# ELEKTRONN/ELEKTRONN2

Hardware: AMD Instinct MI355X
Metric: training_input_voxels_per_sec (higher is better)
Workload: dtype f32; 1 GPU; neuro3d_lite (1,1,23,183,183)->(1,2,10,37,37) fwd+bwd+Adam, 1 sample/GPU; parallelism=dp1, hipgraph=True, steps_per_launch=10

## Files before the change

elektronn2_amd/autotune.py:

```python
from __future__ import annotations

import json
import math
import os

from . import tiling
from .backend import E2Error

_HERE = os.path.dirname(os.path.abspath(__file__))
_SHIPPED = os.path.join(_HERE, "tuned.json")
_cache = None
_dirty = False
IGEMM_MTS = [1, 2, 3, 4, 5, 6, 7, 8, 10, 13]
WGRAD_MTS = [1, 2, 3, 4, 5, 7]


def _cache_path():
    return os.environ.get("E2HIP_TUNE_CACHE", os.path.join(_HERE, ".tune_cache.json"))


def _load():
    global _cache
    if _cache is None:
        _cache = {}
# ... 153 lines not shown
                    if g > 1 and (tiles <= n_cu or wm * wn > 6):
                        continue
                    cands.append("4,%d,%d,%d,%d,%d,%d,%d" % (mg, nt, cc, sk, wm, wn, g))
    return cands


def wgrad_candidates(cout, cin, k, out_sp, n_cu=256):
    mblocks = -(-cout // 16)
    T = k[0] * k[1] * k[2]
    nblocks = -(-(cin * T) // 16)
    q = out_sp[1] * out_sp[2]
    qpad = out_sp[1] * (out_sp[2] + 2 * (k[2] - 1))
    cands = []
    for mt in _best_mts(mblocks, WGRAD_MTS, keep=3):
        nmt = -(-mblocks // mt)
        variants = [(1, 1), (2, 1), (4, 1), (2, 14), (4, 14), (1, 0), (2, 0), (4, 0)]
        if nblocks <= 2:
            variants = [(1, 4), (1, 0), (1, 1), (2, 14)]
        for nt, wk in variants:
            wn = 1 if wk in (4, 14) else 4
            if nt > 1 and 16 * nt * wn > 16 * nblocks:
                continue
            nnt = -(-nblocks // (nt * wn))
            for bp in ((128, 256) if wk in (1, 14) else (64, 128)):
                tiles = out_sp[0] * (-(-(qpad if wk in (1, 14) else q) // bp))
                for fill in (1, 1.5, 2, 3, 4):
                    ps = max(1, min(tiles, int(n_cu * fill) // max(1, nmt * nnt)))
                    for q in {ps} | set(_near_divisors(tiles, ps)):
                        cands.append("%d,%d,%d,%d,%d" % (mt, nt, wk, bp, q))
                        if wk in (1, 14) and nnt >= 2 and nmt * q * nnt > 8:
                            cands.append("%d,%d,%d,%d,%d" % (mt, nt, wk + 100, bp, q))
    return sorted(set(cands) | set(pointwise_wgrad_candidates(cout, cin, k, out_sp, n_cu))
                  | set(position_split_wgrad_candidates(cout, cin, k, out_sp, n_cu))
                  | set(even_split_wgrad_candidates(cout, cin, k, out_sp, n_cu)))


WGRAD_KS_TILES = [(13, 2), (10, 2), (8, 2), (8, 4), (7, 2), (7, 4), (6, 4), (5, 4), (4, 4), (3, 4), (2, 4)]


def position_split_wgrad_candidates(cout, cin, k, out_sp, n_cu=256):
    T = k[0] * k[1] * k[2]
    if T == 1 or cout < 24:
        return []
    pitch = out_sp[2] + k[2] - 1
    if (k[1] - 1) * pitch + k[2] - 1 < 31:
        return []
    units = out_sp[0] * (-(-((out_sp[1] - 1) * pitch + out_sp[2]) // 32))
    scored = []
    for mt, nt in WGRAD_KS_TILES:
        nm, nn = -(-cout // (16 * mt)), -(-(cin * T) // (16 * nt))
        eff = (cout * cin * T) / float(nm * 16 * mt * nn * 16 * nt)
        scored.append((-eff, -mt * nt, mt, nt, nm * nn))
    scored.sort()
    out = []
    for _, _, mt, nt, tiles in scored[:4]:
        for fill in (0.5, 1, 2):
            s = max(1, min(-(-units // 4), int(n_cu * fill) // tiles))
            out.append("%d,%d,9,0,%d" % (mt, nt, s))
    return sorted(set(out))


def even_split_wgrad_candidates(cout, cin, k, out_sp, n_cu=256):
    T = k[0] * k[1] * k[2]
    if T == 1:
        if cout < 32 or cin < 32 or out_sp[0] * out_sp[1] * out_sp[2] < 32:
            return []
        tiles, form = PW_WGRAD_KS_TILES, 8
# ... 193 lines not shown
```

elektronn2_amd/csrc/conv_host.hpp:

```cpp
#pragma once
#include <stdint.h>
#include <string.h>
#include "../../include/e2hip.h"

constexpr int kE2TilingChars = 64;
struct E2Tiling {
  int n = 0;
  int v[8] = {};
};

static inline bool e2_parse_tiling(const char* s, E2Tiling* out) {
  E2Tiling t;
  *out = t;
  if (!s[0]) return true;
  if (strlen(s) >= (size_t)kE2TilingChars) return false;
  for (;;) {
    if (t.n == 8) return false;
    const bool neg = *s == '-';
    if (neg) ++s;
    if (*s < '0' || *s > '9') return false;
    int64_t x = 0;
    for (; *s >= '0' && *s <= '9'; ++s) {
      x = x * 10 + (*s - '0');
      if (x > INT32_MAX) return false;
// ... 78 lines not shown
  int kd = 0, kh = 0, kw = 0;
  int Do = 0, Ho = 0, Wo = 0;
  int64_t xsN = 0, xsC = 0, xsZ = 0, xsY = 0;
  int64_t dsN = 0, dsC = 0, dsZ = 0, dsY = 0;
  int flip = 0;
  int upR = 1;
  int accumulate = 0;
  int dy_padded = 0;
};

static inline WgradArgs wgrad_args(const e2_tensor5& x, const e2_tensor5& dy, float* dw, int kd,
                                   int kh, int kw, int accumulate, int dy_padded) {
  WgradArgs a;
  a.x = x.ptr; a.dy = dy.ptr; a.dw = dw;
  a.N = x.n; a.Cin = x.c; a.Cout = dy.c;
  a.kd = kd; a.kh = kh; a.kw = kw;
  a.Do = dy.d; a.Ho = dy.h; a.Wo = dy.w;
  a.xsN = x.sn; a.xsC = x.sc; a.xsZ = x.sd; a.xsY = x.sh;
  a.dsN = dy.sn; a.dsC = dy.sc; a.dsZ = dy.sd; a.dsY = dy.sh;
  a.flip = 1;
  a.accumulate = accumulate; a.dy_padded = dy_padded;
  return a;
}

enum E2WgradFamily { E2_WG_LDS, E2_WG_DIRECT, E2_WG_PW, E2_WG_PW_KS, E2_WG_KS };
struct E2WgradRoute {
  int family = E2_WG_LDS;
  int MT = 0, NT = 0;
  int BP = 0;
  bool wave_split = false;
  bool xcd = false;
  int splits = 0;
  int bands = 0, groups = 0;
  const char* refuse = nullptr;
};
static inline E2WgradRoute e2_wgrad_route(const int v[5], bool dy_padded) {
  E2WgradRoute r;
  const int WK = v[2], BP = v[3];
  r.MT = v[0]; r.NT = v[1]; r.splits = v[4];
  if (WK == 7) { r.family = E2_WG_PW; return r; }
  if (WK == 8 || WK == 9) {
    r.family = WK == 8 ? E2_WG_PW_KS : E2_WG_KS;
    if (BP >= 1) { r.bands = BP; r.groups = v[4]; }
    return r;
  }
  r.BP = BP;
  if (dy_padded && (WK == 1 || WK == 14 || WK == 101 || WK == 114) && (BP == 128 || BP == 256)) {
    r.family = E2_WG_DIRECT; r.wave_split = WK % 100 == 14; r.xcd = WK >= 100;
    return r;
  }
  if (WK == 14 || WK >= 100) r.refuse = "wgrad: WK=14/101/114 need the padded-gradient entry point and BP 128/256";
  else if (BP != 64 && BP != 128) r.refuse = "wgrad: BP must be 64 or 128";
  else if (!(WK == 0 || WK == 1 || (WK == 4 && r.NT == 1))) r.refuse = "wgrad: WK=4 needs NT=1";
  else r.wave_split = WK == 4;
  return r;
}
static inline const char* e2_wgrad_family_name(const E2WgradRoute& r, bool bf16) {
  switch (r.family) {
    case E2_WG_PW: return "pw_wgrad";
    case E2_WG_PW_KS: return "pw_wgrad_ks";
    case E2_WG_KS: return "wgrad_ks";
    case E2_WG_DIRECT: return bf16 ? "wgrad_direct_bf16r" : "wgrad_direct";
  }
  return "wgrad_lds";
}

static inline const char* e2_pw_wgrad_limit(const WgradArgs& a, bool bf16, int ) {
  if (!(a.kd == 1 && a.kh == 1 && a.kw == 1)) return "pointwise wgrad: the kernel is not 1x1x1";
  if (!(a.xsY == a.Wo && a.xsZ == (int64_t)a.Ho * a.Wo && a.dsY == a.Wo && a.dsZ == (int64_t)a.Ho * a.Wo))
    return "pointwise wgrad: x and dy need dense channel planes (row stride = W, plane stride = H * W)";
  if (bf16) return "pointwise wgrad: an f32 kernel, not offered in bf16 mode";
  return nullptr;
}
static inline const char* e2_wgrad_ks_limit(const WgradArgs& a, bool bf16, int input_slack) {
  const int64_t Din = a.Do + a.kd - 1, Hin = a.Ho + a.kh - 1;
// ... 25 lines not shown
```

elektronn2_amd/csrc/conv_pw_wgrad.hip:

```cpp
#include "common.hpp"
#include "wgrad_even.hpp"
#include <algorithm>
#include <type_traits>
#include <vector>
#include <cstdio>

typedef float f32x4 __attribute__((ext_vector_type(4)));

#ifdef E2_DEBUG_ENV
#define KS_STAMP(i) do { if (p.stamps && threadIdx.x == 0) p.stamps[8L * blockIdx.x + (i)] = __builtin_amdgcn_s_memtime(); } while (0)
#else
#define KS_STAMP(i) do {} while (0)
#endif

namespace {

struct PgP {
  const float* a; const float* b; float* c;
  long asN, asC, bsN, bsC;
  int N, M, Ncol, K;
  int R;
  int nMT, nNT, S;
  int stepsPerSample, steps, per;
  int rem;
  int T, kh, kw, flip, planes;
  long asZ, bsZ, bsY;
  unsigned long long* stamps;
};

__device__ __forceinline__ f32x4 pg_load(const float* row, int k, int K) {
  if (k + 3 < K) {
    f32x4 v;
    __builtin_memcpy(&v, row + k, 16);
    return v;
  }
  f32x4 v = {0.f, 0.f, 0.f, 0.f};
#pragma unroll
  for (int j = 0; j < 4; ++j)
    if (k + j < K) v[j] = row[k + j];
  return v;
}

template <int MT, int NT>
__global__ __launch_bounds__(256) void pw_wgrad_kernel(PgP p) {
  const int tid = threadIdx.x, lane = tid & 63, l15 = lane & 15, q = lane >> 4;
  const int wave = __builtin_amdgcn_readfirstlane(tid >> 6);
  const int wm = wave >> 1, wn = wave & 1;
  int b = blockIdx.x;
  const int nt = b % p.nNT; b /= p.nNT;
  const int mt = b % p.nMT;
  const int sp = b / p.nMT;
  const int m0 = (mt * 2 + wm) * 16 * MT;
  const int n0 = (nt * 2 + wn) * 16 * NT;
  const int s0 = sp * p.per, s1 = min(s0 + p.per, p.steps);

  long aoff[MT], boff[NT];
#pragma unroll
  for (int mb = 0; mb < MT; ++mb) aoff[mb] = (long)min(m0 + 16 * mb + l15, p.M - 1) * p.asC;
#pragma unroll
  for (int nb = 0; nb < NT; ++nb) boff[nb] = (long)min(n0 + 16 * nb + l15, p.Ncol - 1) * p.bsC;

  f32x4 acc[MT][NT];
#pragma unroll
  for (int mb = 0; mb < MT; ++mb)
#pragma unroll
    for (int nb = 0; nb < NT; ++nb) acc[mb][nb] = f32x4{0.f, 0.f, 0.f, 0.f};

  auto load = [&](int s, f32x4 (&A)[MT], f32x4 (&B)[NT]) {
    const int sc = min(s, s1 - 1);
    const int n = sc / p.stepsPerSample;
    const int k = (sc - n * p.stepsPerSample) * 16 + 4 * q;
    const float* ap = p.a + (long)n * p.asN;
    const float* bp = p.b + (long)n * p.bsN;
#pragma unroll
    for (int mb = 0; mb < MT; ++mb) A[mb] = pg_load(ap + aoff[mb], k, p.K);
// ... 22 lines not shown
        load(s + d + D - 1, A[(d + D - 1) % D], B[(d + D - 1) % D]);
        fma(A[d], B[d]);
      }
    }
#pragma unroll
    for (int d = 0; d < D - 1; ++d)
      if (s + d < s1) fma(A[d], B[d]);
  }

  const bool single = p.S == 1;
#pragma unroll
  for (int mb = 0; mb < MT; ++mb) {
#pragma unroll
    for (int r = 0; r < 4; ++r) {
      const int m = m0 + 16 * mb + 4 * q + r;
      if (m >= p.M) continue;
      long rbase;
      int cstride;
      if (p.R > 1) { const int co = m / p.R; rbase = (long)co * p.Ncol * p.R + (m - co * p.R); cstride = p.R; }
      else { rbase = (long)m * p.Ncol; cstride = 1; }
#pragma unroll
      for (int nb = 0; nb < NT; ++nb) {
        const int n = n0 + 16 * nb + l15;
        if (n >= p.Ncol) continue;
        float* dst = p.c + rbase + (long)n * cstride;
        if (single) *dst += acc[mb][nb][r];
        else unsafeAtomicAdd(dst, acc[mb][nb][r]);
      }
    }
  }
}

template <int MT, int NT, bool TAPS>
__global__ __launch_bounds__(256) void pw_wgrad_ks_kernel(PgP p) {
  extern __shared__ float red[];
  constexpr int RW = 16 * NT + 4;
  constexpr int RS = 16 * MT * RW;
  const int tid = threadIdx.x, lane = tid & 63, l15 = lane & 15, q = lane >> 4;
  const int wave = __builtin_amdgcn_readfirstlane(tid >> 6);
  int L = blockIdx.x;
  if ((gridDim.x & 7) == 0) L = (L & 7) * (gridDim.x >> 3) + (L >> 3);
  const int nt = L % p.nNT; L /= p.nNT;
  const int mt = L % p.nMT;
  const int sp = L / p.nMT;
  const int m0 = mt * 16 * MT, n0 = nt * 16 * NT;
  const bool single = p.S == 1;
  auto dst_of = [&](int m, int n) -> float* {
    if (p.R > 1) { const int co = m / p.R; return p.c + (long)co * p.Ncol * p.R + (m - co * p.R) + (long)n * p.R; }
    return p.c + (long)m * p.Ncol + n;
  };

  if (sp >= p.S) return;
  const int u0 = sp * p.per + wave, u1 = min(sp * p.per + p.per, p.steps);
  const int cnt = u0 < u1 ? (u1 - u0 + 3) >> 2 : 0;
  KS_STAMP(0);

  unsigned aoff[MT], boff[NT];
#pragma unroll
  for (int mb = 0; mb < MT; ++mb) aoff[mb] = (unsigned)min(m0 + 16 * mb + l15, p.M - 1) * (unsigned)p.asC * 4u + 16u * q;
#pragma unroll
  for (int nb = 0; nb < NT; ++nb) {
    const int j = min(n0 + 16 * nb + l15, p.Ncol - 1);
    if (TAPS) {
      const int ci = j / p.T, ts = j - ci * p.T;
      const int t = p.flip ? p.T - 1 - ts : ts;
      const int tz = t / (p.kh * p.kw), r2 = t - tz * (p.kh * p.kw);
// ... 5 lines not shown
    }
  }

  f32x4 acc[MT][NT];
#pragma unroll
  for (int mb = 0; mb < MT; ++mb)
#pragma unroll
    for (int nb = 0; nb < NT; ++nb) acc[mb][nb] = f32x4{0.f, 0.f, 0.f, 0.f};

  auto where = [&](int i, const char*& ap, const char*& bp, unsigned& kb, unsigned& zb) {
    const int u = u0 + 4 * i;
    const int pl = u / p.stepsPerSample;
    kb = (unsigned)(u - pl * p.stepsPerSample) * 128u;
    if (TAPS) {
      const int n = pl / p.planes, z = pl - n * p.planes;
      ap = reinterpret_cast<const char*>(p.a + (long)n * p.asN + (long)z * p.asZ);
      bp = reinterpret_cast<const char*>(p.b + (long)n * p.bsN);
      zb = (unsigned)(z * p.bsZ) * 4u;
    } else {
      ap = reinterpret_cast<const char*>(p.a + (long)pl * p.asN);
      bp = reinterpret_cast<const char*>(p.b + (long)pl * p.bsN);
      zb = 0;
    }
  };
  auto bo = [&](int nb, unsigned kb, unsigned zb) -> unsigned {
    return TAPS ? boff[nb] + zb + kb : boff[nb] + kb;
  };
  auto load2 = [&](f32x4 (&d)[2], const char* base, unsigned off) {
    const char* r = base + off;
    __builtin_memcpy(&d[0], r, 16);
    __builtin_memcpy(&d[1], r + 64, 16);
  };

  if (cnt > 0) {
    f32x4 A[MT][2], Bc[NT][2], Bn[NT][2];
    const char *ap, *bp;
    unsigned kb, zb;
    where(0, ap, bp, kb, zb);
#pragma unroll
    for (int nb = 0; nb < NT; ++nb) load2(Bc[nb], bp, bo(nb, kb, zb));
#pragma unroll
    for (int mb = 0; mb < MT; ++mb) load2(A[mb], ap, aoff[mb] + kb);
    KS_STAMP(1);
#pragma unroll 1
    for (int i = 0; i < cnt; ++i) {
      where(min(i + 1, cnt - 1), ap, bp, kb, zb);
#pragma unroll
      for (int nb = 0; nb < NT; ++nb) load2(Bn[nb], bp, bo(nb, kb, zb));
#pragma unroll
      for (int mb = 0; mb < MT; ++mb) {
#pragma unroll
        for (int h = 0; h < 2; ++h)
#pragma unroll
          for (int j = 0; j < 4; ++j)
#pragma unroll
            for (int nb = 0; nb < NT; ++nb)
              acc[mb][nb] = __builtin_amdgcn_mfma_f32_16x16x4f32(A[mb][h][j], Bc[nb][h][j], acc[mb][nb], 0, 0, 0);
        load2(A[mb], ap, aoff[mb] + kb);
        __builtin_amdgcn_sched_barrier(0);
      }
#pragma unroll
      for (int nb = 0; nb < NT; ++nb) { Bc[nb][0] = Bn[nb][0]; Bc[nb][1] = Bn[nb][1]; }
#ifdef E2_DEBUG_ENV
      if (i == 0) KS_STAMP(2);
#endif
    }
  }
// ... 26 lines not shown
#pragma unroll
            for (int nb = 0; nb < NT; ++nb)
              acc[mb][nb] = __builtin_amdgcn_mfma_f32_16x16x4f32(av[mb >> 2][e], bv[nb][e], acc[mb][nb], 0, 0, 0);
        }
    }
  }

  float* mine = red + wave * RS;
#pragma unroll
  for (int mb = 0; mb < MT; ++mb)
#pragma unroll
    for (int nb = 0; nb < NT; ++nb)
#pragma unroll
      for (int r = 0; r < 4; ++r) mine[(16 * mb + 4 * q + r) * RW + 16 * nb + l15] = acc[mb][nb][r];
  __syncthreads();
  KS_STAMP(4);
#pragma unroll 2
  for (int e = tid; e < 16 * MT * 16 * NT; e += 256) {
    const int ml = e / (16 * NT), nl = e - ml * (16 * NT);
    const int m = m0 + ml, n = n0 + nl;
    const float* s = red + ml * RW + nl;
    const float v = (s[0] + s[RS]) + (s[2 * RS] + s[3 * RS]);
    if (m >= p.M || n >= p.Ncol) continue;
    float* dst = dst_of(m, n);
    if (single) *dst += v;
    else unsafeAtomicAdd(dst, v);
  }
  KS_STAMP(5);
#ifdef E2_DEBUG_ENV
  if (p.stamps) { __builtin_amdgcn_s_waitcnt(0); KS_STAMP(6); }
#endif
}

template <int MT, int NT, bool TAPS>
__global__ __launch_bounds__(256) void pw_wgrad_ev_kernel(PgP p, WgEven ev) {
  extern __shared__ float red[];
  constexpr int RW = 16 * NT + 4;
  constexpr int RS = 16 * MT * RW;
  const int tid = threadIdx.x, lane = tid & 63, l15 = lane & 15, q = lane >> 4;
  const int wave = __builtin_amdgcn_readfirstlane(tid >> 6);
  int g = blockIdx.x;
  if ((ev.G & 7) == 0) g = (g & 7) * (ev.G >> 3) + (g >> 3);
  WgRange rg = wg_even_range(ev, g);
  if (rg.b >= rg.e) return;
  KS_STAMP(0);
#ifdef E2_DEBUG_ENV
  int nseg = 0;
#endif
#pragma unroll 1
  do {
    const WgSeg sg = wg_even_seg(ev, rg);
    const int mt = sg.tile / p.nNT, nt = sg.tile - mt * p.nNT;
    const int m0 = mt * 16 * MT, n0 = nt * 16 * NT;
    const int u0 = sg.u0 + wave, u1 = sg.u0 + sg.n;
    const int cnt = u0 < u1 ? (u1 - u0 + 3) >> 2 : 0;

    unsigned aoff[MT], boff[NT];
#pragma unroll
    for (int mb = 0; mb < MT; ++mb) aoff[mb] = (unsigned)min(m0 + 16 * mb + l15, p.M - 1) * (unsigned)p.asC * 4u + 16u * q;
#pragma unroll
    for (int nb = 0; nb < NT; ++nb) {
      const int j = min(n0 + 16 * nb + l15, p.Ncol - 1);
      if (TAPS) {
        const int ci = j / p.T, ts = j - ci * p.T;
        const int t = p.flip ? p.T - 1 - ts : ts;
        const int tz = t / (p.kh * p.kw), r2 = t - tz * (p.kh * p.kw);
        const int ty = r2 / p.kw, tx = r2 - ty * p.kw;
// ... 4 lines not shown
      }
    }

    f32x4 acc[MT][NT];
#pragma unroll
    for (int mb = 0; mb < MT; ++mb)
#pragma unroll
      for (int nb = 0; nb < NT; ++nb) acc[mb][nb] = f32x4{0.f, 0.f, 0.f, 0.f};

    auto where = [&](int i, const char*& ap, const char*& bp, unsigned& kb, unsigned& zb) {
      const int u = u0 + 4 * i;
      const int pl = u / p.stepsPerSample;
      kb = (unsigned)(u - pl * p.stepsPerSample) * 128u;
      if (TAPS) {
        const int n = pl / p.planes, z = pl - n * p.planes;
        ap = reinterpret_cast<const char*>(p.a + (long)n * p.asN + (long)z * p.asZ);
        bp = reinterpret_cast<const char*>(p.b + (long)n * p.bsN);
        zb = (unsigned)(z * p.bsZ) * 4u;
      } else {
        ap = reinterpret_cast<const char*>(p.a + (long)pl * p.asN);
        bp = reinterpret_cast<const char*>(p.b + (long)pl * p.bsN);
        zb = 0;
      }
    };
    auto bo = [&](int nb, unsigned kb, unsigned zb) -> unsigned {
      return TAPS ? boff[nb] + zb + kb : boff[nb] + kb;
    };
    auto load2 = [&](f32x4 (&d)[2], const char* base, unsigned off) {
      const char* r = base + off;
      __builtin_memcpy(&d[0], r, 16);
      __builtin_memcpy(&d[1], r + 64, 16);
    };

    if (cnt > 0) {
      f32x4 A[MT][2], Bc[NT][2], Bn[NT][2];
      const char *ap, *bp;
      unsigned kb, zb;
      where(0, ap, bp, kb, zb);
#pragma unroll
      for (int nb = 0; nb < NT; ++nb) load2(Bc[nb], bp, bo(nb, kb, zb));
#pragma unroll
      for (int mb = 0; mb < MT; ++mb) load2(A[mb], ap, aoff[mb] + kb);
#pragma unroll 1
      for (int i = 0; i < cnt; ++i) {
        where(min(i + 1, cnt - 1), ap, bp, kb, zb);
#pragma unroll
        for (int nb = 0; nb < NT; ++nb) load2(Bn[nb], bp, bo(nb, kb, zb));
#pragma unroll
        for (int mb = 0; mb < MT; ++mb) {
#pragma unroll
          for (int h = 0; h < 2; ++h)
#pragma unroll
            for (int j = 0; j < 4; ++j)
#pragma unroll
              for (int nb = 0; nb < NT; ++nb)
                acc[mb][nb] = __builtin_amdgcn_mfma_f32_16x16x4f32(A[mb][h][j], Bc[nb][h][j], acc[mb][nb], 0, 0, 0);
          load2(A[mb], ap, aoff[mb] + kb);
          __builtin_amdgcn_sched_barrier(0);
        }
#pragma unroll
        for (int nb = 0; nb < NT; ++nb) { Bc[nb][0] = Bn[nb][0]; Bc[nb][1] = Bn[nb][1]; }
      }
    }
    if (!TAPS && u1 == ev.U && p.rem > 0) {
      constexpr int MBW = (MT + 3) / 4;
      const int k = p.K - p.rem + 4 * q;
#pragma unroll 1
// ... 30 lines not shown
    for (int mb = 0; mb < MT; ++mb)
#pragma unroll
      for (int nb = 0; nb < NT; ++nb)
#pragma unroll
        for (int r = 0; r < 4; ++r) mine[(16 * mb + 4 * q + r) * RW + 16 * nb + l15] = acc[mb][nb][r];
    __syncthreads();
#pragma unroll 2
    for (int e = tid; e < 16 * MT * 16 * NT; e += 256) {
      const int ml = e / (16 * NT), nl = e - ml * (16 * NT);
      const int m = m0 + ml, n = n0 + nl;
      const float* s = red + ml * RW + nl;
      const float v = (s[0] + s[RS]) + (s[2 * RS] + s[3 * RS]);
      if (m >= p.M || n >= p.Ncol) continue;
      float* dst;
      if (p.R > 1) { const int co = m / p.R; dst = p.c + (long)co * p.Ncol * p.R + (m - co * p.R) + (long)n * p.R; }
      else dst = p.c + (long)m * p.Ncol + n;
      unsafeAtomicAdd(dst, v);
    }
    __syncthreads();
#ifdef E2_DEBUG_ENV
    ++nseg;
#endif
    rg.b += sg.n;
  } while (rg.b < rg.e);
#ifdef E2_DEBUG_ENV
  if (p.stamps) {
    __builtin_amdgcn_s_waitcnt(0);
    KS_STAMP(6);
    if (threadIdx.x == 0) p.stamps[8L * blockIdx.x + 7] = (unsigned long long)nseg;
  }
#endif
}

template <int MT, int NT, bool TAPS>
int launch_ev(e2_ctx* ctx, const PgP& p, const WgEven& ev) {
  const int lds = 4 * 16 * MT * (16 * NT + 4) * (int)sizeof(float);
  static bool raised = false;
  if (int rc = e2i_raise_lds(reinterpret_cast<const void*>(&pw_wgrad_ev_kernel<MT, NT, TAPS>), lds, &raised)) return rc;
  PgP ps = p;
#ifdef E2_DEBUG_ENV
  const long grid = ev.G;
  const bool stamps = e2_dbg_env("E2_PWKS_STAMPS") != nullptr && !ctx->capturing;
  if (stamps) {
    E2_CHECK_HIP(hipMalloc(&ps.stamps, sizeof(unsigned long long) * 8 * grid));
    E2_CHECK_HIP(hipMemsetAsync(ps.stamps, 0, sizeof(unsigned long long) * 8 * grid, ctx->stream));
  }
#endif
  hipLaunchKernelGGL((pw_wgrad_ev_kernel<MT, NT, TAPS>), dim3((unsigned)ev.G), dim3(256), lds, ctx->stream, ps, ev);
  E2_CHECK_HIP(hipGetLastError());
#ifdef E2_DEBUG_ENV
  if (stamps) {
    E2_CHECK_HIP(hipStreamSynchronize(ctx->stream));
    std::vector<unsigned long long> h(8 * grid);
    E2_CHECK_HIP(hipMemcpy(h.data(), ps.stamps, sizeof(unsigned long long) * 8 * grid, hipMemcpyDeviceToHost));
    unsigned long long t0 = ~0ull, t1 = 0;
    double sum[2] = {0, 0}, mx[2] = {0, 0};
    long cntw[2] = {0, 0};
    for (long b = 0; b < grid; ++b) {
      if (!h[8 * b + 6]) continue;
      const int k = h[8 * b + 7] > 1;
      const double d = (double)(h[8 * b + 6] - h[8 * b]);
      sum[k] += d; mx[k] = std::max(mx[k], d); ++cntw[k];
      t0 = std::min(t0, h[8 * b]); t1 = std::max(t1, h[8 * b + 6]);
    }
    fprintf(stderr, "[e2] pw_wgrad_ev<%d,%d> G %d, %d tiles x %d units in %d bands, %d(+1 for %d) pairs each: first start -> last end %llu ticks\n",
            MT, NT, ev.G, ev.T, ev.U, ev.B, ev.base, ev.extra, t1 - t0);
    for (int k = 0; k < 2; ++k)
      fprintf(stderr, "   %-22s %5ld work-groups, mean %9.0f max %9.0f ticks\n", k ? "two or more segments" : "one segment",
              cntw[k], sum[k] / std::max(1L, cntw[k]), mx[k]);
    (void)hipFree(ps.stamps);
  }
#endif
  return 0;
}

static int even_split(const PgP& p, long G, int B, WgEven* ev) {
  const long T = (long)p.nMT * p.nNT;
  E2_REQUIRE(p.steps >= 1, "wgrad (even position ranges): no whole 32-position unit");
  E2_REQUIRE(T * p.steps < (1L << 31), "wgrad (even position ranges): too many (tile, unit) pairs");
  E2_REQUIRE(G >= 1 && G <= (1L << 16), "wgrad (even position ranges): %ld work-groups (1 .. 65536)", G);
  E2_REQUIRE(B >= 1 && B <= p.steps, "wgrad (even position ranges): %d bands for %d units", B, p.steps);
  *ev = wg_even_make((int)T, p.steps, (int)G, B);
  return 0;
}

template <int MT, int NT, bool TAPS>
int launch_ks(e2_ctx* ctx, const PgP& p, long grid) {
  const int lds = 4 * 16 * MT * (16 * NT + 4) * (int)sizeof(float);
  static bool raised = false;
  if (int rc = e2i_raise_lds(reinterpret_cast<const void*>(&pw_wgrad_ks_kernel<MT, NT, TAPS>), lds, &raised)) return rc;
#ifdef E2_DEBUG_ENV
  PgP ps = p;
  const bool stamps = e2_dbg_env("E2_PWKS_STAMPS") != nullptr && !ctx->capturing;
  if (stamps) {
    E2_CHECK_HIP(hipMalloc(&ps.stamps, sizeof(unsigned long long) * 8 * grid));
    E2_CHECK_HIP(hipMemsetAsync(ps.stamps, 0, sizeof(unsigned long long) * 8 * grid, ctx->stream));
  }
  hipLaunchKernelGGL((pw_wgrad_ks_kernel<MT, NT, TAPS>), dim3((unsigned)grid), dim3(256), lds, ctx->stream, ps);
  E2_CHECK_HIP(hipGetLastError());
  if (stamps) {
    E2_CHECK_HIP(hipStreamSynchronize(ctx->stream));
    std::vector<unsigned long long> h(8 * grid);
    E2_CHECK_HIP(hipMemcpy(h.data(), ps.stamps, sizeof(unsigned long long) * 8 * grid, hipMemcpyDeviceToHost));
    static const char* names[6] = {"prologue issue", "first unit", "other units", "LDS + barrier", "flush issue", "flush done"};
    double sum[6] = {0};
    unsigned long long t0 = ~0ull, t1 = 0, s1 = 0;
    long nb = 0;
    for (long b = 0; b < grid; ++b) {
      if (!h[8 * b + 6]) continue;
      ++nb;
      for (int i = 0; i < 6; ++i) sum[i] += (double)(h[8 * b + i + 1] - h[8 * b + i]);
      t0 = std::min(t0, h[8 * b]); t1 = std::max(t1, h[8 * b + 6]); s1 = std::max(s1, h[8 * b]);
    }
    fprintf(stderr, "[e2] pw_wgrad_ks<%d,%d> grid %ld (%ld main), S %d, per %d: first start -> last end %llu ticks, last start %llu\n",
            MT, NT, grid, nb, p.S, p.per, t1 - t0, s1 - t0);
    for (int i = 0; i < 6; ++i) fprintf(stderr, "   %-14s %9.0f ticks\n", names[i], sum[i] / std::max(1L, nb));
    (void)hipFree(ps.stamps);
  }
#else
  hipLaunchKernelGGL((pw_wgrad_ks_kernel<MT, NT, TAPS>), dim3((unsigned)grid), dim3(256), lds, ctx->stream, p);
  E2_CHECK_HIP(hipGetLastError());
#endif
  return 0;
}

template <int MT, int NT>
int launch(e2_ctx* ctx, const PgP& p, long grid) {
  hipLaunchKernelGGL((pw_wgrad_kernel<MT, NT>), dim3((unsigned)grid), dim3(256), 0, ctx->stream, p);
  E2_CHECK_HIP(hipGetLastError());
  return 0;
}

PgP pg_base(const WgradArgs& a, int Ncol, long K) {
  PgP p;
  p.a = a.dy; p.b = a.x; p.c = a.dw;
  p.asN = a.dsN; p.asC = a.dsC; p.bsN = a.xsN; p.bsC = a.xsC;
  p.N = a.N; p.M = a.Cout; p.Ncol = Ncol;
  p.K = (int)K;
  p.R = 1; p.rem = 0; p.stamps = nullptr;
  p.T = 1; p.kh = p.kw = 1; p.flip = 0; p.planes = 1; p.asZ = p.bsZ = p.bsY = 0;
  return p;
}

struct KsSplit { long grid; bool even; WgEven ev; };
int ks_split(e2_ctx* ctx, const WgradArgs& a, const E2WgradRoute& r, long units, const char* who, PgP& p, KsSplit* k) {
  E2_REQUIRE(units < (1L << 29), "%s: too many positions", who);
  p.steps = (int)units;
  const int S = (int)std::max<long>(1, std::min<long>(r.splits, std::max<long>(1, (units + 3) / 4)));
  p.per = (int)std::max<long>(1, (units + S - 1) / S);
  p.per = (p.per + 3) & ~3;
  p.S = (int)std::max<long>(1, (units + p.per - 1) / p.per);
  k->grid = (long)p.nMT * p.nNT * p.S;
  k->grid = (k->grid + 7) & ~7L;
  E2_REQUIRE(k->grid < (1L << 31), "%s: grid too large", who);
  k->even = r.bands >= 1;
  k->ev = WgEven{};
  if (k->even)
    if (int rc = even_split(p, r.groups, r.bands, &k->ev)) return rc;
  if (!a.accumulate)
    if (int rc = e2i_fill_flat(ctx, a.dw, (size_t)a.Cout * p.Ncol, 0.f)) return rc;
  return 0;
}
template <int MT, int NT, bool TAPS>
int launch_split(e2_ctx* ctx, const PgP& p, const KsSplit& k) {
  return k.even ? launch_ev<MT, NT, TAPS>(ctx, p, k.ev) : launch_ks<MT, NT, TAPS>(ctx, p, k.grid);
}

}

int e2i_pw_wgrad(e2_ctx* ctx, const WgradArgs& a, const E2WgradRoute& r) {
  const char* limit = e2_pw_wgrad_limit(a, ctx->mfma_bf16 != 0, ctx->input_slack);
  E2_REQUIRE(!limit, "%s", limit);
  const long K = (long)a.Do * a.Ho * a.Wo;
  E2_REQUIRE(K < (1L << 30), "pointwise wgrad: sample too large");
  PgP p = pg_base(a, a.Cin, K);
  p.R = a.upR > 1 ? a.upR : 1;
  E2_REQUIRE(a.Cout % p.R == 0, "pointwise wgrad: %d rows for %d sub-positions", a.Cout, p.R);
  p.nMT = e2_cdiv(a.Cout, 32 * r.MT);
  p.nNT = e2_cdiv(a.Cin, 32 * r.NT);
  p.stepsPerSample = (int)((K + 15) / 16);
  const long steps = (long)a.N * p.stepsPerSample;
  E2_REQUIRE(steps < (1L << 30), "pointwise wgrad: too many positions");
  p.steps = (int)steps;
  const int S = (int)std::max<long>(1, std::min<long>(r.splits, steps));
  p.per = (int)((steps + S - 1) / S);
  p.S = (int)((steps + p.per - 1) / p.per);
  const long grid = (long)p.nMT * p.nNT * p.S;
  E2_REQUIRE(grid < (1L << 31), "pointwise wgrad: grid too large");
  if (!a.accumulate)
    if (int rc = e2i_fill_flat(ctx, a.dw, (size_t)a.Cout * a.Cin, 0.f)) return rc;
#define E2_L(M, N_) if (r.MT == M && r.NT == N_) return launch<M, N_>(ctx, p, grid);
  E2_L(2, 2) E2_L(4, 2) E2_L(2, 4) E2_L(4, 4) E2_L(4, 3) E2_L(3, 4) E2_L(7, 2) E2_L(2, 7) E2_L(7, 4) E2_L(4, 7)
#undef E2_L
  e2_set_error("pointwise wgrad: no instance MT=%d NT=%d", r.MT, r.NT);
  return 2;
}

int e2i_pw_wgrad_ks(e2_ctx* ctx, const WgradArgs& a, const E2WgradRoute& r) {
  const char* limit = e2_pw_wgrad_limit(a, ctx->mfma_bf16 != 0, ctx->input_slack);
  E2_REQUIRE(!limit, "%s", limit);
  const long K = (long)a.Do * a.Ho * a.Wo;
  E2_REQUIRE(K >= 4 && K < (1L << 30), "pointwise wgrad: sample of %ld positions", K);
  E2_REQUIRE(((long)a.Cout * a.dsC + K) * 4 < (1L << 32) && ((long)a.Cin * a.xsC + K) * 4 < (1L << 32) && a.dsC >= 0 && a.xsC >= 0,
             "pointwise wgrad: sample too large for 32-bit byte offsets");
  PgP p = pg_base(a, a.Cin, K);
  p.R = a.upR > 1 ? a.upR : 1;
  E2_REQUIRE(a.Cout % p.R == 0, "pointwise wgrad: %d rows for %d sub-positions", a.Cout, p.R);
  p.nMT = e2_cdiv(a.Cout, 16 * r.MT);
  p.nNT = e2_cdiv(a.Cin, 16 * r.NT);
  p.stepsPerSample = (int)(K / 32);
  p.rem = (int)(K % 32);
  KsSplit k;
  if (int rc = ks_split(ctx, a, r, (long)a.N * p.stepsPerSample, "pointwise wgrad", p, &k)) return rc;
#define E2_L(M, N_) if (r.MT == M && r.NT == N_) return launch_split<M, N_, false>(ctx, p, k);
  E2_L(13, 2) E2_L(7, 2) E2_L(7, 4) E2_L(4, 4) E2_L(10, 2)
#undef E2_L
  e2_set_error("pointwise wgrad (position-split waves): no instance MT=%d NT=%d", r.MT, r.NT);
  return 2;
}

int e2i_wgrad_ks(e2_ctx* ctx, const WgradArgs& a, const E2WgradRoute& r) {
  const char* limit = e2_wgrad_ks_limit(a, ctx->mfma_bf16 != 0, ctx->input_slack);
  E2_REQUIRE(!limit, "%s", limit);
  const int T = a.kd * a.kh * a.kw;
  const long K = (long)(a.Ho - 1) * a.dsY + a.Wo;
  E2_REQUIRE(K >= 4 && K < (1L << 28), "wgrad (position-split GEMM): plane of %ld positions", K);
  PgP p = pg_base(a, a.Cin * T, K);
  p.T = T; p.kh = a.kh; p.kw = a.kw; p.flip = a.flip; p.planes = a.Do;
  p.asZ = a.dsZ; p.bsZ = a.xsZ; p.bsY = a.xsY;
#ifdef E2_DEBUG_ENV
  if (!ctx->capturing) {
    const int Din = a.Do + a.kd - 1, Hin = a.Ho + a.kh - 1;
    const float* end = a.x + (int64_t)(a.N - 1) * a.xsN + (int64_t)(a.Cin - 1) * a.xsC +
                       (int64_t)(Din - 1) * a.xsZ + (int64_t)(Hin - 1) * a.xsY + (a.Wo + a.kw - 1);
    float h[32];
    E2_CHECK_HIP(hipStreamSynchronize(ctx->stream));
    E2_CHECK_HIP(hipMemcpy(h, end, sizeof(h), hipMemcpyDeviceToHost));
    for (int i = 0; i < 32; ++i)
      E2_REQUIRE(h[i] == h[i] && h[i] - h[i] == 0.f, "wgrad (position-split GEMM): e2_set_input_slack promised finite "
                 "values behind x, but float %d behind its last element is %g", i, (double)h[i]);
  }
#endif
  p.nMT = e2_cdiv(a.Cout, 16 * r.MT);
  p.nNT = e2_cdiv(p.Ncol, 16 * r.NT);
  p.stepsPerSample = (int)((K + 31) / 32);
  KsSplit k;
  if (int rc = ks_split(ctx, a, r, (long)a.N * a.Do * p.stepsPerSample, "wgrad (position-split GEMM)", p, &k)) return rc;
#define E2_L(M, N_) if (r.MT == M && r.NT == N_) return launch_split<M, N_, true>(ctx, p, k);
  E2_L(13, 2) E2_L(7, 2) E2_L(7, 4) E2_L(4, 4) E2_L(10, 2) E2_L(5, 4) E2_L(3, 4) E2_L(2, 4) E2_L(8, 2) E2_L(8, 4) E2_L(6, 4)
#undef E2_L
  e2_set_error("wgrad (position-split GEMM): no instance MT=%d NT=%d", r.MT, r.NT);
  return 2;
}
```

elektronn2_amd/csrc/conv_wgrad.hip:

```cpp
#include "wgrad_common.hpp"
#include <stdlib.h>
#include <utility>

struct WgradP {
  const float* x;
  const float* dy;
  const float* zeros;
  float* dw;
  int Cin, Cout, kd, kh, kw, T, THW;
  int Do, Ho, Wo, Q;
  long xsN, xsC, xsZ, xsY;
  long dsN, dsC, dsZ, dsY;
  int flip, upR;
  int NTOT;
  int Lpad;
  int nMT, nNT, nPS;
  int nPT, tilesTotal;
  int maxSpans;
  int bufFloats;
  int Din, N;
  int dbg;
  int bf16;
  FastDiv divWo;
};
// ... 251 lines not shown
  e2_set_error("wgrad: no instance NT=%d BP=%d WK=%d", NT, BP, WK);
  return 2;
}

static int w_lpad(int Lmax) {
  return ((Lmax + 63) / 64) * 64 + 2;
}
static int w_lmax(const WgradArgs& a, int BP) {
  const int rows = (BP + a.Wo - 2) / a.Wo;
  return (BP - 1) + rows * ((int)a.xsY - a.Wo) + (a.kh - 1) * (int)a.xsY + a.kw;
}
static size_t w_buf_floats(const WgradArgs& a, int MT, int BNn, int BP) {
  const size_t dyf = (((size_t)16 * MT * (BP + 4) + 3) / 4) * 4;
  return dyf + (BP + 128) + (size_t)wg_maxspans(a, BNn) * w_lpad(w_lmax(a, BP)) + 64;
}

struct WCfg { int MT, NT, WK, BP, PS; };

static WCfg choose_wcfg(const e2_ctx* ctx, const WgradArgs& a, int* ok, int* src) {
  const int mblocks = e2_cdiv(a.Cout, 16);
  const int T = a.kd * a.kh * a.kw;
  const long NTOT = (long)a.Cin * T;
  const int nblocks = (int)((NTOT + 15) / 16);
  const long Q = (long)a.Ho * a.Wo;
  WCfg best{0, 0, 0, 0, 0};
  double bestCost = 1e300;
  const double dw_bytes = 4.0 * a.Cout * (double)NTOT;
  const E2Tiling& t = ctx->tiling_v[E2_TILING_WGRAD];
  *src = E2_SRC_MODEL;
  if (t.n) {
    *src = E2_SRC_FALLBACK;
    if (e2_wgrad_candidate(t)) {
      const WCfg f{t.v[0], t.v[1], t.v[2], t.v[3], t.v[4]};
      const char* limit = f.WK == 9 ? e2_wgrad_ks_limit(a, ctx->mfma_bf16, ctx->input_slack)
                          : (f.WK == 7 || f.WK == 8) ? e2_pw_wgrad_limit(a, ctx->mfma_bf16, ctx->input_slack)
                          : nullptr;
      if (limit == nullptr) { *ok = 1; *src = E2_SRC_FORCED; return f; }
    }
  }
  if (a.dy_padded && nblocks > 2) {
    const long S = (long)(a.Ho - 1) * a.dsY + a.Wo;
    for (int MT : kWgMTs) {
      if (MT > mblocks && MT != 1) continue;
      const int nMT = e2_cdiv(mblocks, MT);
      for (int NT = 1; NT <= 4; NT *= 2) {
        if (16 * NT * 4 > 16 * nblocks && NT > 1) continue;
        if (NT == 4 && MT * 4 >= 20) continue;
        const int nNT = e2_cdiv(nblocks, NT * 4);
        for (int BP = ctx->mfma_bf16 ? 256 : 128; BP <= 256; BP *= 2) {
          if (BP == 256 && S <= 128 && !ctx->mfma_bf16) continue;
          const size_t lds = 2 * e2i_wgrad_direct_buf_floats(a, NT, BP, 1) * 4;
          if (lds > 160 * 1024) continue;
          const int slots = ctx->num_cu;
          const int nPT = (int)((S + BP - 1) / BP);
          const long tiles = (long)a.N * a.Do * nPT;
          const long base = (long)nMT * nNT;
          for (int fill = 1; fill <= 2; ++fill) {
            long PS = std::max<long>(1, ((long)slots * fill + base - 1) / base);
            PS = std::min(PS, tiles);
            const int per = (int)((tiles + PS - 1) / PS);
            const double tile = (BP / 4.0) * MT * NT * 35.0 + (BP / 16.0) * 150.0 + 1200.0;
            const double flush = 16.0 * MT * 16.0 * NT * 4 * 0.6;
            const double wg_time = per * tile + flush + 5000.0;
            const long wgs = base * PS;
            const double rounds = (double)((wgs + slots - 1) / slots);
            const double atom = (double)PS * dw_bytes / 1.3e12 * 2.4e9 + dw_bytes / 4e12 * 2.4e9;
            const double cost = rounds * wg_time + atom;
            if (cost < bestCost) { bestCost = cost; best = WCfg{MT, NT, 1, BP, (int)PS}; }
// ... 96 lines not shown
```

elektronn2_amd/tiling.py:

```python
import re
from collections import namedtuple

_LIST = re.compile(r"-?[0-9]+(,-?[0-9]+){0,7}")


WgradRoute = namedtuple('WgradRoute', 'family MT NT WK BP wave_split xcd splits bands groups refuse')


class Tiling(namedtuple('Tiling', 'kind family v')):
    __slots__ = ()

    @property
    def WK(self):
        return wgrad_route(self, True).WK if self.family == 'wgrad' else None

    @property
    def xcd_grouped(self):
        return self.family == 'wgrad' and wgrad_route(self, True).xcd


def wgrad_route(t, dy_padded, bf16=False):
    assert t.kind == 'wgrad' and t.family == 'wgrad', t
    MT, NT, WK, BP, PS = t.v
    r = dict(family='wgrad_lds', MT=MT, NT=NT, WK=WK, BP=0, wave_split=False, xcd=False, splits=PS,
             bands=0, groups=0, refuse=None)
    if WK == 7:
        r.update(family='pw_wgrad')
    elif WK in (8, 9):
        r.update(family='pw_wgrad_ks' if WK == 8 else 'wgrad_ks')
        if BP >= 1:
            r.update(bands=BP, groups=PS)
    elif dy_padded and WK in (1, 14, 101, 114) and BP in (128, 256):
        r.update(family='wgrad_direct_bf16r' if bf16 else 'wgrad_direct', BP=BP,
                 wave_split=WK % 100 == 14, xcd=WK >= 100)
    else:
        r.update(BP=BP)
        if WK == 14 or WK >= 100:
            r.update(refuse="WK=14/101/114 need the padded-gradient entry point and BP 128/256")
        elif BP not in (64, 128):
            r.update(refuse="BP must be 64 or 128")
        elif not (WK in (0, 1) or (WK == 4 and NT == 1)):
            r.update(refuse="WK=4 needs NT=1")
        else:
            r.update(wave_split=WK == 4)
    return WgradRoute(**r)


def parse(kind, s):
    if not s or len(s) > 63 or not _LIST.fullmatch(s):
        return None
    v = tuple(int(t) for t in s.split(","))
    if any(abs(q) >= 2 ** 31 for q in v):
        return None
    fam = None
    if kind == 'igemm':
        if len(v) == 4:
            fam = '16x16x4'
        elif len(v) == 8 and v[0] == 4:
            fam = '4x4x1'
        elif len(v) in (3, 5) and v[0] == 1:
            fam = 'pointwise'
        elif len(v) >= 3 and v[0] == 32:
# ... 46 lines not shown
```

Measured before the change: 528.4 million voxels/s.

## Add six-product bf16-split wgrad variant for position-split and pointwise kernels

Adds a new wgrad kernel variant (WK=18/19) that splits each fp32 operand into three bf16 pieces and accumulates six bf16 MFMA cross-products. This gives near-fp32 accuracy on the bf16 matrix cores without the bf16 input limit checks. The new candidates are added to the autotuner's search space and routed through the existing ks/even launch paths. The cost is six MFMAs per k-step plus the splitting arithmetic, so it only helps where the autotuner finds it beats the existing fp32 paths.

```diff
diff --git a/elektronn2_amd/autotune.py b/elektronn2_amd/autotune.py
--- a/elektronn2_amd/autotune.py
+++ b/elektronn2_amd/autotune.py
@@ -209,7 +209,22 @@
                             cands.append("%d,%d,%d,%d,%d" % (mt, nt, wk + 100, bp, q))
     return sorted(set(cands) | set(pointwise_wgrad_candidates(cout, cin, k, out_sp, n_cu))
                   | set(position_split_wgrad_candidates(cout, cin, k, out_sp, n_cu))
-                  | set(even_split_wgrad_candidates(cout, cin, k, out_sp, n_cu)))
+                  | set(even_split_wgrad_candidates(cout, cin, k, out_sp, n_cu))
+                  | set(six_product_wgrad_candidates(cout, cin, k, out_sp, n_cu)))
+
+
+def six_product_form(c):
+    v = c.split(",")
+    if len(v) == 5 and v[2] in ("8", "9"):
+        return ",".join(v[:2] + ["1" + v[2]] + v[3:])
+    return None
+
+
+def six_product_wgrad_candidates(cout, cin, k, out_sp, n_cu=256):
+    out = []
+    for gen in (pointwise_wgrad_candidates, position_split_wgrad_candidates, even_split_wgrad_candidates):
+        out += [six_product_form(c) for c in gen(cout, cin, k, out_sp, n_cu)]
+    return sorted(set(c for c in out if c))
 
 
 WGRAD_KS_TILES = [(13, 2), (10, 2), (8, 2), (8, 4), (7, 2), (7, 4), (6, 4), (5, 4), (4, 4), (3, 4), (2, 4)]
diff --git a/elektronn2_amd/csrc/conv_host.hpp b/elektronn2_amd/csrc/conv_host.hpp
--- a/elektronn2_amd/csrc/conv_host.hpp
+++ b/elektronn2_amd/csrc/conv_host.hpp
@@ -134,6 +134,7 @@
   bool xcd = false;
   int splits = 0;
   int bands = 0, groups = 0;
+  bool six = false;
   const char* refuse = nullptr;
 };
 static inline E2WgradRoute e2_wgrad_route(const int v[5], bool dy_padded) {
@@ -141,8 +142,9 @@
   const int WK = v[2], BP = v[3];
   r.MT = v[0]; r.NT = v[1]; r.splits = v[4];
   if (WK == 7) { r.family = E2_WG_PW; return r; }
-  if (WK == 8 || WK == 9) {
-    r.family = WK == 8 ? E2_WG_PW_KS : E2_WG_KS;
+  if (WK == 8 || WK == 9 || WK == 18 || WK == 19) {
+    r.family = WK % 10 == 8 ? E2_WG_PW_KS : E2_WG_KS;
+    r.six = WK >= 18;
     if (BP >= 1) { r.bands = BP; r.groups = v[4]; }
     return r;
   }
diff --git a/elektronn2_amd/csrc/conv_pw_wgrad.hip b/elektronn2_amd/csrc/conv_pw_wgrad.hip
--- a/elektronn2_amd/csrc/conv_pw_wgrad.hip
+++ b/elektronn2_amd/csrc/conv_pw_wgrad.hip
@@ -41,6 +41,38 @@
   return v;
 }
 
+typedef __bf16 bf16x8 __attribute__((ext_vector_type(8)));
+typedef unsigned u32x4 __attribute__((ext_vector_type(4)));
+typedef float f32x2 __attribute__((ext_vector_type(2)));
+struct Pc3 { u32x4 p[3]; };
+
+__device__ __forceinline__ Pc3 pg_split8(const f32x4 (&d)[2]) {
+  Pc3 f;
+#pragma unroll
+  for (int h = 0; h < 2; ++h)
+#pragma unroll
+    for (int e = 0; e < 2; ++e) {
+      f32x2 r = {d[h][2 * e], d[h][2 * e + 1]};
+#pragma unroll
+      for (int pc = 0; pc < 3; ++pc) {
+        const unsigned t0 = __float_as_uint(r[0]) & 0xffff0000u, t1 = __float_as_uint(r[1]) & 0xffff0000u;
+        f.p[pc][2 * h + e] = (t0 >> 16) | t1;
+        if (pc < 2) r -= f32x2{__uint_as_float(t0), __uint_as_float(t1)};
+      }
+    }
+  return f;
+}
+template <int NT>
+__device__ __forceinline__ void pg_mfma6(const Pc3& a, const Pc3 (&b)[NT], f32x4 (&acc)[NT]) {
+  constexpr int TA[6] = {1, 0, 2, 0, 1, 0}, TB[6] = {1, 2, 0, 1, 0, 0};
+#pragma unroll
+  for (int t = 0; t < 6; ++t)
+#pragma unroll
+    for (int nb = 0; nb < NT; ++nb)
+      acc[nb] = __builtin_amdgcn_mfma_f32_16x16x32_bf16(__builtin_bit_cast(bf16x8, a.p[TA[t]]),
+                                                        __builtin_bit_cast(bf16x8, b[nb].p[TB[t]]), acc[nb], 0, 0, 0);
+}
+
 template <int MT, int NT>
 __global__ __launch_bounds__(256) void pw_wgrad_kernel(PgP p) {
   const int tid = threadIdx.x, lane = tid & 63, l15 = lane & 15, q = lane >> 4;
@@ -129,6 +161,75 @@
 }
 
 template <int MT, int NT, bool TAPS>
+__device__ __forceinline__ void pg_six_units(const PgP& p, int u0, int cnt, const unsigned (&aoff)[MT],
+                                             const unsigned (&boff)[NT], f32x4 (&acc)[MT][NT]) {
+  auto where = [&](int i, const char*& ap, const char*& bp, unsigned& kb, unsigned& zb) {
+    const int u = u0 + 4 * i;
+    const int pl = u / p.stepsPerSample;
+    kb = (unsigned)(u - pl * p.stepsPerSample) * 128u;
+    if (TAPS) {
+      const int n = pl / p.planes, z = pl - n * p.planes;
+      ap = reinterpret_cast<const char*>(p.a + (long)n * p.asN + (long)z * p.asZ);
+      bp = reinterpret_cast<const char*>(p.b + (long)n * p.bsN);
+      zb = (unsigned)(z * p.bsZ) * 4u;
+    } else {
+      ap = reinterpret_cast<const char*>(p.a + (long)pl * p.asN);
+      bp = reinterpret_cast<const char*>(p.b + (long)pl * p.bsN);
+      zb = 0;
+    }
+  };
+  auto bo = [&](int nb, unsigned kb, unsigned zb) -> unsigned {
+    return TAPS ? boff[nb] + zb + kb : boff[nb] + kb;
+  };
+  auto load2 = [&](f32x4 (&d)[2], const char* base, unsigned off) {
+    const char* r = base + off;
+    __builtin_memcpy(&d[0], r, 16);
+    __builtin_memcpy(&d[1], r + 64, 16);
+  };
+  f32x4 A[MT][2], Bn[NT][2];
+  Pc3 Ap, Bp[NT];
+  const char *ap, *bp;
+  unsigned kb, zb;
+  where(0, ap, bp, kb, zb);
+#pragma unroll
+  for (int nb = 0; nb < NT; ++nb) load2(Bn[nb], bp, bo(nb, kb, zb));
+#pragma unroll
+  for (int mb = 0; mb < MT; ++mb) load2(A[mb], ap, aoff[mb] + kb);
+#pragma unroll
+  for (int nb = 0; nb < NT; ++nb) Bp[nb] = pg_split8(Bn[nb]);
+  Ap = pg_split8(A[0]);
+  where(min(1, cnt - 1), ap, bp, kb, zb);
+#pragma unroll
+  for (int nb = 0; nb < NT; ++nb) load2(Bn[nb], bp, bo(nb, kb, zb));
+  load2(A[0], ap, aoff[0] + kb);
+#pragma unroll 1
+  for (int i = 0; i < cnt; ++i) {
+    Pc3 Bq[NT];
+#pragma unroll
+    for (int mb = 0; mb < MT; ++mb) {
+      Pc3 An;
+      if (mb + 1 < MT) {
+        An = pg_split8(A[mb + 1]);
+        load2(A[mb + 1], ap, aoff[mb + 1] + kb);
+      } else {
+        An = pg_split8(A[0]);
+#pragma unroll
+        for (int nb = 0; nb < NT; ++nb) Bq[nb] = pg_split8(Bn[nb]);
+        where(min(i + 2, cnt - 1), ap, bp, kb, zb);
+#pragma unroll
+        for (int nb = 0; nb < NT; ++nb) load2(Bn[nb], bp, bo(nb, kb, zb));
+        load2(A[0], ap, aoff[0] + kb);
+      }
+      pg_mfma6<NT>(Ap, Bp, acc[mb]);
+      Ap = An;
+      __builtin_amdgcn_sched_barrier(0);
+    }
+#pragma unroll
+    for (int nb = 0; nb < NT; ++nb) Bp[nb] = Bq[nb];
+  }
+}
+
+template <int MT, int NT, bool TAPS, bool SIX = false>
 __global__ __launch_bounds__(256) void pw_wgrad_ks_kernel(PgP p) {
   extern __shared__ float red[];
   constexpr int RW = 16 * NT + 4;
@@ -200,7 +301,9 @@
     __builtin_memcpy(&d[1], r + 64, 16);
   };
 
-  if (cnt > 0) {
+  if constexpr (SIX) {
+    if (cnt > 0) pg_six_units<MT, NT, TAPS>(p, u0, cnt, aoff, boff, acc);
+  } else if (cnt > 0) {
     f32x4 A[MT][2], Bc[NT][2], Bn[NT][2];
     const char *ap, *bp;
     unsigned kb, zb;
@@ -293,7 +396,7 @@
 #endif
 }
 
-template <int MT, int NT, bool TAPS>
+template <int MT, int NT, bool TAPS, bool SIX = false>
 __global__ __launch_bounds__(256) void pw_wgrad_ev_kernel(PgP p, WgEven ev) {
   extern __shared__ float red[];
   constexpr int RW = 16 * NT + 4;
@@ -364,7 +467,9 @@
       __builtin_memcpy(&d[1], r + 64, 16);
     };
 
-    if (cnt > 0) {
+    if constexpr (SIX) {
+      if (cnt > 0) pg_six_units<MT, NT, TAPS>(p, u0, cnt, aoff, boff, acc);
+    } else if (cnt > 0) {
       f32x4 A[MT][2], Bc[NT][2], Bn[NT][2];
       const char *ap, *bp;
       unsigned kb, zb;
@@ -461,11 +566,11 @@
 #endif
 }
 
-template <int MT, int NT, bool TAPS>
+template <int MT, int NT, bool TAPS, bool SIX>
 int launch_ev(e2_ctx* ctx, const PgP& p, const WgEven& ev) {
   const int lds = 4 * 16 * MT * (16 * NT + 4) * (int)sizeof(float);
   static bool raised = false;
-  if (int rc = e2i_raise_lds(reinterpret_cast<const void*>(&pw_wgrad_ev_kernel<MT, NT, TAPS>), lds, &raised)) return rc;
+  if (int rc = e2i_raise_lds(reinterpret_cast<const void*>(&pw_wgrad_ev_kernel<MT, NT, TAPS, SIX>), lds, &raised)) return rc;
   PgP ps = p;
 #ifdef E2_DEBUG_ENV
   const long grid = ev.G;
@@ -475,7 +580,7 @@
     E2_CHECK_HIP(hipMemsetAsync(ps.stamps, 0, sizeof(unsigned long long) * 8 * grid, ctx->stream));
   }
 #endif
-  hipLaunchKernelGGL((pw_wgrad_ev_kernel<MT, NT, TAPS>), dim3((unsigned)ev.G), dim3(256), lds, ctx->stream, ps, ev);
+  hipLaunchKernelGGL((pw_wgrad_ev_kernel<MT, NT, TAPS, SIX>), dim3((unsigned)ev.G), dim3(256), lds, ctx->stream, ps, ev);
   E2_CHECK_HIP(hipGetLastError());
 #ifdef E2_DEBUG_ENV
   if (stamps) {
@@ -513,11 +618,11 @@
   return 0;
 }
 
-template <int MT, int NT, bool TAPS>
+template <int MT, int NT, bool TAPS, bool SIX>
 int launch_ks(e2_ctx* ctx, const PgP& p, long grid) {
   const int lds = 4 * 16 * MT * (16 * NT + 4) * (int)sizeof(float);
   static bool raised = false;
-  if (int rc = e2i_raise_lds(reinterpret_cast<const void*>(&pw_wgrad_ks_kernel<MT, NT, TAPS>), lds, &raised)) return rc;
+  if (int rc = e2i_raise_lds(reinterpret_cast<const void*>(&pw_wgrad_ks_kernel<MT, NT, TAPS, SIX>), lds, &raised)) return rc;
 #ifdef E2_DEBUG_ENV
   PgP ps = p;
   const bool stamps = e2_dbg_env("E2_PWKS_STAMPS") != nullptr && !ctx->capturing;
@@ -525,7 +630,7 @@
     E2_CHECK_HIP(hipMalloc(&ps.stamps, sizeof(unsigned long long) * 8 * grid));
     E2_CHECK_HIP(hipMemsetAsync(ps.stamps, 0, sizeof(unsigned long long) * 8 * grid, ctx->stream));
   }
-  hipLaunchKernelGGL((pw_wgrad_ks_kernel<MT, NT, TAPS>), dim3((unsigned)grid), dim3(256), lds, ctx->stream, ps);
+  hipLaunchKernelGGL((pw_wgrad_ks_kernel<MT, NT, TAPS, SIX>), dim3((unsigned)grid), dim3(256), lds, ctx->stream, ps);
   E2_CHECK_HIP(hipGetLastError());
   if (stamps) {
     E2_CHECK_HIP(hipStreamSynchronize(ctx->stream));
@@ -547,7 +652,7 @@
     (void)hipFree(ps.stamps);
   }
 #else
-  hipLaunchKernelGGL((pw_wgrad_ks_kernel<MT, NT, TAPS>), dim3((unsigned)grid), dim3(256), lds, ctx->stream, p);
+  hipLaunchKernelGGL((pw_wgrad_ks_kernel<MT, NT, TAPS, SIX>), dim3((unsigned)grid), dim3(256), lds, ctx->stream, p);
   E2_CHECK_HIP(hipGetLastError());
 #endif
   return 0;
@@ -591,8 +696,9 @@
   return 0;
 }
 template <int MT, int NT, bool TAPS>
-int launch_split(e2_ctx* ctx, const PgP& p, const KsSplit& k) {
-  return k.even ? launch_ev<MT, NT, TAPS>(ctx, p, k.ev) : launch_ks<MT, NT, TAPS>(ctx, p, k.grid);
+int launch_split(e2_ctx* ctx, const PgP& p, const KsSplit& k, bool six) {
+  if (six) return k.even ? launch_ev<MT, NT, TAPS, true>(ctx, p, k.ev) : launch_ks<MT, NT, TAPS, true>(ctx, p, k.grid);
+  return k.even ? launch_ev<MT, NT, TAPS, false>(ctx, p, k.ev) : launch_ks<MT, NT, TAPS, false>(ctx, p, k.grid);
 }
 
 }
@@ -641,7 +747,7 @@
   p.rem = (int)(K % 32);
   KsSplit k;
   if (int rc = ks_split(ctx, a, r, (long)a.N * p.stepsPerSample, "pointwise wgrad", p, &k)) return rc;
-#define E2_L(M, N_) if (r.MT == M && r.NT == N_) return launch_split<M, N_, false>(ctx, p, k);
+#define E2_L(M, N_) if (r.MT == M && r.NT == N_) return launch_split<M, N_, false>(ctx, p, k, r.six);
   E2_L(13, 2) E2_L(7, 2) E2_L(7, 4) E2_L(4, 4) E2_L(10, 2)
 #undef E2_L
   e2_set_error("pointwise wgrad (position-split waves): no instance MT=%d NT=%d", r.MT, r.NT);
@@ -675,7 +781,7 @@
   p.stepsPerSample = (int)((K + 31) / 32);
   KsSplit k;
   if (int rc = ks_split(ctx, a, r, (long)a.N * a.Do * p.stepsPerSample, "wgrad (position-split GEMM)", p, &k)) return rc;
-#define E2_L(M, N_) if (r.MT == M && r.NT == N_) return launch_split<M, N_, true>(ctx, p, k);
+#define E2_L(M, N_) if (r.MT == M && r.NT == N_) return launch_split<M, N_, true>(ctx, p, k, r.six);
   E2_L(13, 2) E2_L(7, 2) E2_L(7, 4) E2_L(4, 4) E2_L(10, 2) E2_L(5, 4) E2_L(3, 4) E2_L(2, 4) E2_L(8, 2) E2_L(8, 4) E2_L(6, 4)
 #undef E2_L
   e2_set_error("wgrad (position-split GEMM): no instance MT=%d NT=%d", r.MT, r.NT);
diff --git a/elektronn2_amd/csrc/conv_wgrad.hip b/elektronn2_amd/csrc/conv_wgrad.hip
--- a/elektronn2_amd/csrc/conv_wgrad.hip
+++ b/elektronn2_amd/csrc/conv_wgrad.hip
@@ -307,8 +307,10 @@
     *src = E2_SRC_FALLBACK;
     if (e2_wgrad_candidate(t)) {
       const WCfg f{t.v[0], t.v[1], t.v[2], t.v[3], t.v[4]};
-      const char* limit = f.WK == 9 ? e2_wgrad_ks_limit(a, ctx->mfma_bf16, ctx->input_slack)
-                          : (f.WK == 7 || f.WK == 8) ? e2_pw_wgrad_limit(a, ctx->mfma_bf16, ctx->input_slack)
+      const bool six = f.WK == 18 || f.WK == 19;
+      const bool bf16 = ctx->mfma_bf16 && !six;
+      const char* limit = (f.WK == 9 || f.WK == 19) ? e2_wgrad_ks_limit(a, bf16, ctx->input_slack)
+                          : (f.WK == 7 || f.WK == 8 || f.WK == 18) ? e2_pw_wgrad_limit(a, bf16, ctx->input_slack)
                           : nullptr;
       if (limit == nullptr) { *ok = 1; *src = E2_SRC_FORCED; return f; }
     }
diff --git a/elektronn2_amd/tiling.py b/elektronn2_amd/tiling.py
--- a/elektronn2_amd/tiling.py
+++ b/elektronn2_amd/tiling.py
@@ -4,7 +4,7 @@
 _LIST = re.compile(r"-?[0-9]+(,-?[0-9]+){0,7}")
 
 
-WgradRoute = namedtuple('WgradRoute', 'family MT NT WK BP wave_split xcd splits bands groups refuse')
+WgradRoute = namedtuple('WgradRoute', 'family MT NT WK BP wave_split xcd splits bands groups refuse six')
 
 
 class Tiling(namedtuple('Tiling', 'kind family v')):
@@ -23,11 +23,11 @@
     assert t.kind == 'wgrad' and t.family == 'wgrad', t
     MT, NT, WK, BP, PS = t.v
     r = dict(family='wgrad_lds', MT=MT, NT=NT, WK=WK, BP=0, wave_split=False, xcd=False, splits=PS,
-             bands=0, groups=0, refuse=None)
+             bands=0, groups=0, refuse=None, six=False)
     if WK == 7:
         r.update(family='pw_wgrad')
-    elif WK in (8, 9):
-        r.update(family='pw_wgrad_ks' if WK == 8 else 'wgrad_ks')
+    elif WK in (8, 9, 18, 19):
+        r.update(family='pw_wgrad_ks' if WK % 10 == 8 else 'wgrad_ks', six=WK >= 18)
         if BP >= 1:
             r.update(bands=BP, groups=PS)
     elif dy_padded and WK in (1, 14, 101, 114) and BP in (128, 256):
```

Result: faster. 554.1 million voxels/s, median of 6 (+4.9%).
